# colinsongf/keyword_spotting

Hardware: NVIDIA B200
Metric: streamed audio-sec/sec, 2L GRU-128 KWS (higher is better)
Workload: dtype f16 operands / f32 accumulate+state

## Files before the change

keyword_spotting_b200/csrc/api.cu:

```cuda
#include <cmath>
#include <cstring>
#include <vector>

#include <cuda_fp16.h>

#include "common.cuh"

namespace kws {

static thread_local std::string g_last_error;

void set_error(const char* fmt, ...) {
  char buf[1024];
  va_list ap;
  va_start(ap, fmt);
  vsnprintf(buf, sizeof(buf), fmt, ap);
  va_end(ap);
  g_last_error = buf;
}
void clear_error() { g_last_error.clear(); }
int fail(int code, const char* fmt, ...) {
  char buf[1024];
  va_list ap;
  va_start(ap, fmt);
// ... 50 lines not shown
  if (m->aux_stream) cudaStreamDestroy(m->aux_stream);
  cudaFree(m->scratch_mel);
  cudaFree(m->scratch_seq);
  cudaFree(m->tc_xt);
  free_octbit(m);
  delete m;
}

}

using namespace kws;

extern "C" const char* kws_last_error(void) { return g_last_error.c_str(); }
extern "C" int kws_abi_version(void) { return KWS_B200_ABI_VERSION; }

extern "C" int kws_device_count(void) {
  clear_error();
  int n = 0;
  cudaError_t e = cudaGetDeviceCount(&n);
  if (e != cudaSuccess) return fail(KWS_ERR_CUDA, "cudaGetDeviceCount failed: %s", cudaGetErrorString(e));
  return n;
}

extern "C" int kws_model_create(const kws_model_config* cfg, const kws_model_weights* w, int device,
                                kws_model** out) {
  clear_error();
  KWS_REQUIRE(cfg && w && out, "NULL argument");
  *out = nullptr;
  KWS_REQUIRE(cfg->hidden == kHidden, "hidden_size must be %d (config/rnn_config.py:84)", kHidden);
  KWS_REQUIRE(cfg->num_layers >= 1 && cfg->num_layers <= kMaxLayers, "num_layers must be in [1, %d]", kMaxLayers);
  KWS_REQUIRE(cfg->num_classes >= 2 && cfg->num_classes <= kMaxClasses, "num_classes must be in [2, %d]", kMaxClasses);
  KWS_REQUIRE(cfg->n_mel >= 1 && cfg->n_mel <= kMaxMel, "n_mel must be in [1, %d]", kMaxMel);
  KWS_REQUIRE(cfg->fft_size == kFft && cfg->hop_size == kHop,
              "the front end is built for fft_size=%d hop_size=%d (config/rnn_config.py:57-58)", kFft, kHop);
  KWS_REQUIRE(w->mel_basis && w->fc_w && w->fc_b, "NULL weight pointer");
  for (int l = 0; l < cfg->num_layers; ++l)
    KWS_REQUIRE(w->gates_kernel[l] && w->gates_bias[l] && w->cand_kernel[l] && w->cand_bias[l],
                "NULL weight pointer for layer %d", l);
  int ndev = 0;
  cudaError_t e = cudaGetDeviceCount(&ndev);
  if (e != cudaSuccess || ndev <= 0)
    return fail(KWS_ERR_CUDA, "no CUDA device available (%s); libkws_b200 has no CPU fallback",
                e == cudaSuccess ? "device count 0" : cudaGetErrorString(e));
  KWS_REQUIRE(device >= 0 && device < ndev, "device %d out of range [0, %d)", device, ndev);
  KWS_CUDA_OK(cudaSetDevice(device));

  kws_model* m = new kws_model();
  m->cfg = *cfg;
  m->device = device;
  m->frontend = default_frontend();
  const int M = cfg->n_mel, H = kHidden, C = cfg->num_classes;
  int rc = upload(&m->mel_basis, w->mel_basis, static_cast<size_t>(kBins) * M);
  {
    std::vector<kws::MelQuad> quads;
    kws::build_mel_quads(w->mel_basis, M, &quads, &m->mel.quads_per_warp);
    if (rc == KWS_OK) rc = upload(&m->mel.quads, quads.data(), quads.size());
  }
  if (rc == KWS_OK) rc = build_frontend_tc_tables(m, w->mel_basis);
  std::vector<float2> tw(20 * 52);
  for (int k2 = 0; k2 < 20; ++k2)
    for (int j = 0; j < 52; ++j) {
      const double a = -2.0 * M_PI * static_cast<double>((j % 20) * k2) / kFft;
      tw[k2 * 52 + j] = make_float2(static_cast<float>(std::cos(a)), static_cast<float>(std::sin(a)));
    }
  if (rc == KWS_OK) rc = upload(&m->twiddle400, tw.data(), tw.size());
  for (int l = 0; l < cfg->num_layers && rc == KWS_OK; ++l) {
    const int in = l == 0 ? M : H;
    m->layer[l].in_dim = in;
    rc = upload(&m->layer[l].gates_kernel, w->gates_kernel[l], static_cast<size_t>(in + H) * 2 * H);
    if (rc == KWS_OK) rc = upload(&m->layer[l].gates_bias, w->gates_bias[l], 2 * H);
    if (rc == KWS_OK) rc = upload(&m->layer[l].cand_kernel, w->cand_kernel[l], static_cast<size_t>(in + H) * H);
    if (rc == KWS_OK) rc = upload(&m->layer[l].cand_bias, w->cand_bias[l], H);
    if (rc == KWS_OK) {
      std::vector<__half> packed;
      const bool last = l == cfg->num_layers - 1;
      const bool split = l == 0 && in <= 64 && gru_tc_can_split(in, last, device);
      if (l == 0 && !gru_tc_layer_fits(in, split, last, device)) m->tc_fits = false;
      pack_tc_weights(w->gates_kernel[l], w->cand_kernel[l], in, split, &packed, &m->layer[l].tc_kx, &m->layer[l].tc_kxw);
      __half* dptr = nullptr;
      rc = upload(&dptr, packed.data(), packed.size());
      m->layer[l].tc_wpack = dptr;
      std::vector<float> fused(3 * H);
      for (int i = 0; i < 2 * H; ++i) fused[i] = w->gates_bias[l][i];
      for (int i = 0; i < H; ++i) fused[2 * H + i] = w->cand_bias[l][i];
      if (rc == KWS_OK) rc = upload(&m->layer[l].tc_bias, fused.data(), fused.size());
    }
  }
  if (rc == KWS_OK) rc = upload(&m->fc_w, w->fc_w, static_cast<size_t>(H) * C);
  if (rc == KWS_OK) rc = upload(&m->fc_b, w->fc_b, C);
  m->fc_w_host.assign(w->fc_w, w->fc_w + static_cast<size_t>(H) * C);
  m->fc_b_host.assign(w->fc_b, w->fc_b + C);
  if (rc != KWS_OK) {
    free_model(m);
    return rc;
  }
  *out = m;
  return KWS_OK;
}

extern "C" int kws_model_destroy(kws_model* m) {
  clear_error();
  if (m) {
    cudaSetDevice(m->device);
    free_model(m);
  }
  return KWS_OK;
}

extern "C" int kws_model_set_precision(kws_model* m, int precision) {
  clear_error();
  KWS_REQUIRE(m != nullptr, "model is NULL");
  KWS_REQUIRE(precision == KWS_PRECISION_FP32 || precision == KWS_PRECISION_TC_FP16, "unknown precision %d", precision);
  m->precision = precision;
// ... 147 lines not shown
```

keyword_spotting_b200/csrc/common.cuh:

```cuda
#pragma once

#include <cuda_runtime.h>
#include <stdint.h>

#include <cstdarg>
#include <cstdio>
#include <string>
#include <vector>

#include "../../include/kws_b200.h"

namespace kws {

constexpr int kHidden = 128;
constexpr int kMaxLayers = 4;
constexpr int kMaxClasses = 16;
constexpr int kFft = 400;
constexpr int kHop = 160;
constexpr int kBins = kFft / 2 + 1;
constexpr int kMaxMel = 128;

void set_error(const char* fmt, ...);
void clear_error();
int fail(int code, const char* fmt, ...);
// ... 19 lines not shown
  } while (0)

inline int64_t ceil_div(int64_t a, int64_t b) { return (a + b - 1) / b; }

__host__ __device__ __forceinline__ int att_frames(int T, int combine) { return combine > 1 ? T / combine + 1 : T; }

constexpr int kAttCoreTcMaxKeys = 400;

struct AttLens {
  const int32_t* lens;
  int T;
  int combine;
  __device__ __forceinline__ int frames_in(long b) const { return lens ? min(max(__ldg(lens + b), 1), T) : T; }
  __device__ __forceinline__ int rows_of(long b) const { return att_frames(frames_in(b), combine); }
  __device__ __forceinline__ bool tile_live(int Tp, long rows, long r0, int tile) const {
    if (!lens) return true;
    const long b0 = r0 / Tp;
    const long rlast = (r0 + tile < rows ? r0 + tile : rows) - 1;
    return r0 - b0 * Tp < rows_of(b0) || (b0 + 1) * Tp <= rlast;
  }
};

int sm_count();

struct LayerWeights {
  int in_dim = 0;
  float* gates_kernel = nullptr;
  float* gates_bias = nullptr;
  float* cand_kernel = nullptr;
  float* cand_bias = nullptr;
  int tc_kx = 0;
  int tc_kxw = 0;
  void* tc_wpack = nullptr;
  float* tc_bias = nullptr;
};

struct OctbitMatrix {
  signed char* wq = nullptr;
  float* obias = nullptr;
  float scale = 0.0f;
  int* cand_count = nullptr;
  unsigned short* cand = nullptr;
  int B = 0, K = 0;
};

struct alignas(16) MelQuad {
  float w[4];
  int mag_off;
  int band_off;
  int pad[2];
};
struct MelSparse {
  MelQuad* quads = nullptr;
  int quads_per_warp = 0;
};

struct FrontendTcTables {
  bool ready = false;
  uint32_t* tw = nullptr;
  void* mel_seg = nullptr;
  float* mel_w = nullptr;
  int mel_nw = 0;
};

}

struct kws_model {
  kws_model_config cfg;
  int device = 0;
  int precision = KWS_PRECISION_TC_FP16;
  int frontend = KWS_FRONTEND_FFT;
  float* mel_basis = nullptr;
  kws::MelSparse mel;
  kws::FrontendTcTables fe_tc;
  float2* twiddle400 = nullptr;
  kws::LayerWeights layer[kws::kMaxLayers];
  float* fc_w = nullptr;
  float* fc_b = nullptr;
  std::vector<float> fc_w_host, fc_b_host;
  int64_t cap_streams = 0;
  int32_t cap_frames = 0;
  float* scratch_mel = nullptr;
  float* scratch_seq = nullptr;
  bool octbit = false;
  kws::OctbitMatrix oct_gates[kws::kMaxLayers], oct_cand[kws::kMaxLayers], oct_fc;
  float* oct_y_rows = nullptr;
  size_t oct_y_cap = 0;
  bool tc_fits = true;
  void* tc_xt = nullptr;
  size_t tc_xt_bytes = 0;
  cudaStream_t aux_stream = nullptr;
  std::vector<cudaEvent_t> aux_events;
};

namespace kws {

struct PcmSource {
  const void* body = nullptr;
  int64_t ld_body = 0;
  int32_t body_len = 0;
  int body_dtype = KWS_PCM_F32;
  const int16_t* head = nullptr;
  int64_t ld_head = 0;
  const int32_t* head_len = nullptr;
};

// ... 60 lines not shown
```

keyword_spotting_b200/csrc/fft400.cuh:

```cuda
#pragma once

#if defined(__CUDACC__)
#define KWS_HD __host__ __device__ __forceinline__
#else
#define KWS_HD inline
#endif

namespace kws {
namespace fft {

struct alignas(8) cpx {
  float re, im;
};

constexpr int kN = 400;
constexpr int kR = 20;
constexpr int kRowStride = 21;
constexpr int kBufSlots = kR * kRowStride;
constexpr int kPairWindow = 560;
constexpr int kBins = kN / 2 + 1;

#if defined(__CUDA_ARCH__)
KWS_HD float2 as_f2(cpx a) { return make_float2(a.re, a.im); }
KWS_HD cpx as_cpx(float2 a) { return cpx{a.x, a.y}; }
// ... 6 lines not shown
KWS_HD cpx cross_sq(cpx a, cpx b) {
  const float2 bs = make_float2(b.im, b.re);
  return as_cpx(__ffma2_rn(bs, bs, __fmul2_rn(as_f2(a), as_f2(a))));
}
#else
KWS_HD cpx cadd(cpx a, cpx b) { return cpx{a.re + b.re, a.im + b.im}; }
KWS_HD cpx csub(cpx a, cpx b) { return cpx{a.re - b.re, a.im - b.im}; }
KWS_HD cpx caxpy(float s, cpx b, cpx a) { return cpx{a.re + s * b.re, a.im + s * b.im}; }
KWS_HD cpx cscale(float s, cpx b) { return cpx{s * b.re, s * b.im}; }
KWS_HD cpx csub_i(cpx a, cpx b) { return cpx{a.re + b.im, a.im - b.re}; }
KWS_HD cpx cadd_i(cpx a, cpx b) { return cpx{a.re - b.im, a.im + b.re}; }
KWS_HD cpx cross_sq(cpx a, cpx b) { return cpx{a.re * a.re + b.im * b.im, a.im * a.im + b.re * b.re}; }
#endif
KWS_HD cpx cmul(cpx a, cpx b) { return cpx{a.re * b.re - a.im * b.im, a.re * b.im + a.im * b.re}; }

KWS_HD void dft4(cpx& a0, cpx& a1, cpx& a2, cpx& a3) {
  const cpx t0 = cadd(a0, a2), t1 = csub(a0, a2), t2 = cadd(a1, a3), t3 = csub(a1, a3);
  a0 = cadd(t0, t2);
  a2 = csub(t0, t2);
  a1 = csub_i(t1, t3);
  a3 = cadd_i(t1, t3);
}

KWS_HD void dft5(cpx& a0, cpx& a1, cpx& a2, cpx& a3, cpx& a4) {
  const float c1 = 0.30901699437494742f;
  const float c2 = -0.80901699437494742f;
  const float s1 = 0.95105651629515357f;
  const float s2 = 0.58778525229247313f;
  const cpx t1 = cadd(a1, a4), t2 = cadd(a2, a3), t3 = csub(a1, a4), t4 = csub(a2, a3);
  const cpx m1 = caxpy(c2, t2, caxpy(c1, t1, a0));
  const cpx m2 = caxpy(c1, t2, caxpy(c2, t1, a0));
  const cpx n1 = caxpy(s2, t4, cscale(s1, t3));
  const cpx n2 = caxpy(-s1, t4, cscale(s2, t3));
  a0 = cadd(cadd(a0, t1), t2);
  a1 = csub_i(m1, n1);
  a4 = cadd_i(m1, n1);
  a2 = csub_i(m2, n2);
  a3 = cadd_i(m2, n2);
}

KWS_HD constexpr int pfa_slot(int k) { return (5 * (k % 4) + 4 * (k % 5)) % 20; }

KWS_HD void dft20_pfa(cpx (&v)[20]) {
#pragma unroll
  for (int n2 = 0; n2 < 5; ++n2)
    dft4(v[(4 * n2) % 20], v[(5 + 4 * n2) % 20], v[(10 + 4 * n2) % 20], v[(15 + 4 * n2) % 20]);
#pragma unroll
  for (int k1 = 0; k1 < 4; ++k1)
    dft5(v[(5 * k1) % 20], v[(5 * k1 + 4) % 20], v[(5 * k1 + 8) % 20], v[(5 * k1 + 12) % 20],
         v[(5 * k1 + 16) % 20]);
}

constexpr int kTwStride = 52;
constexpr int kTwSlots = kR * kTwStride;
KWS_HD constexpr int tw_base(int warp, int lane) { return (12 * warp) % kR + lane; }

KWS_HD void stage1_col(int n1, cpx (&v)[20], const cpx* tw, cpx* buf) {
  dft20_pfa(v);
  buf[n1 * kRowStride] = v[pfa_slot(0)];
#pragma unroll
  for (int k2 = 1; k2 < kR; ++k2) buf[n1 * kRowStride + k2] = cmul(v[pfa_slot(k2)], tw[k2 * kTwStride]);
}

KWS_HD void stage2_col(int k2, cpx* buf, cpx (&v)[20]) {
#pragma unroll
  for (int n1 = 0; n1 < kR; ++n1) v[n1] = buf[n1 * kRowStride + k2];
  dft20_pfa(v);
#pragma unroll
  for (int k1 = kR / 2; k1 < kR; ++k1) buf[k1 * kRowStride + k2] = v[pfa_slot(k1)];
}

KWS_HD float sqrt_fast(float x) {
#if defined(__CUDA_ARCH__)
  float r;
  asm("sqrt.approx.ftz.f32 %0, %1;" : "=f"(r) : "f"(x));
  return r;
#else
  return __builtin_sqrtf(x);
#endif
}

KWS_HD void untangle_col(int k2, const cpx (&v)[20], const cpx* buf, float* mag_a, float* mag_b, int k1_stride) {
  const int mcol = k2 == 0 ? 0 : kR - k2;
  const int mrow0 = k2 == 0 ? kR : kR - 1;
#pragma unroll
  for (int k1 = 0; k1 < kR / 2; ++k1) {
    const cpx zk = v[pfa_slot(k1)];
    int mrow = mrow0 - k1;
    const bool self = mrow == kR;
    if (self) mrow = kR - 1;
    cpx zm = buf[mrow * kRowStride + mcol];
    if (self) zm = zk;
    const cpx sp = cadd(zk, zm), sm = csub(zk, zm);
    const cpx sq = cross_sq(sp, sm);
    mag_a[k1 * k1_stride] = sqrt_fast(sq.re);
    mag_b[k1 * k1_stride] = sqrt_fast(sq.im);
  }
  if (k2 == 0) {
    const cpx z = v[pfa_slot(kR / 2)];
    mag_a[(kR / 2) * k1_stride] = 2.0f * (z.re < 0.0f ? -z.re : z.re);
    mag_b[(kR / 2) * k1_stride] = 2.0f * (z.im < 0.0f ? -z.im : z.im);
  }
}

}
}
```

keyword_spotting_b200/csrc/frontend.cu:

```cuda
#include <algorithm>
#include <cstring>
#include <vector>

#include "common.cuh"
#include "tc05.cuh"
#include "fft400.cuh"

namespace kws {

using fft::cpx;

constexpr int kFePairs = 16;
constexpr int kFeThreads = kFePairs * fft::kR;
constexpr int kFeWarps = kFeThreads / 32;
constexpr int kFeItemFrames = 2 * kFePairs;
constexpr int kFeBlock = 2 * kHop;
constexpr int kFeSkew = 20;
constexpr int kFeWinSamples = kFePairs * kFeBlock + (kFft - kHop);
constexpr int kFeWinRounds = (kFeWinSamples + kFeThreads - 1) / kFeThreads;
constexpr int kFeQuadRounds = (kFeWinSamples + 4 * kFeThreads - 1) / (4 * kFeThreads);
constexpr int kFeLastQuads = (kFeWinSamples - 4 * kFeThreads * (kFeQuadRounds - 1)) / 4;
static_assert(kFeWinSamples % 4 == 0 && kFeBlock % 4 == 0, "quads must not straddle a skew boundary");
constexpr int kFeQuadSmemMax = 512;
constexpr int kFeItemHop = kFePairs * kFeBlock;
constexpr int kFeMagStride = 66;
constexpr int kFeWinFloats = kFeWinRounds * (kFeBlock + kFeSkew);
constexpr int kFeMagRows = (fft::kBins + 3) / 2;
constexpr int kFeMagFloats = kFeMagRows * kFeMagStride;
constexpr int kFeMagLive = (fft::kBins / 2) * kFeMagStride;
constexpr int kFeRegionFloats = kFeMagFloats > kFeWinFloats ? kFeMagFloats : kFeWinFloats;
static_assert(kFeWinFloats <= kFeMagLive, "the window must not reach the rows that hold the zero bins");
static_assert((kFeRegionFloats * 4) % 16 == 0, "mel quads follow the region and are read as float4");

struct FrontendParams {
  PcmSource src;
  long S;
  int max_frames;
  int groups;
  const int* nframes;
  int n_mel;
  const cpx* twiddle;
  const MelQuad* mel_q;
  int mel_qpw;
  int vec_ok;
  float* mel_out;
  int tiled_out;
  int tile_chunks;
  int tile_split;
  unsigned c_magic;
  unsigned q_magic;
  float mag_scale;
  int fuse_pre;
  long long vad_limit;
  int16_t* tail_next;
  int* len_next;
  unsigned char* silence;
  int* nframes_out;
};

__device__ __forceinline__ int mag_slot(int pair, int fr) { return ((10 * pair) & 15) + 16 * (pair >> 3) + fr; }
__device__ __forceinline__ int slot_frame(int slot) {
  const int pair = ((5 * ((slot & 15) >> 1)) & 7) + 8 * (slot >> 4);
  return 2 * pair + (slot & 1);
}
__device__ __forceinline__ int mag_index(int bin, int slot) { return (bin >> 1) * kFeMagStride + 2 * slot + (bin & 1); }

__device__ __forceinline__ float4 quad_to_float(uint2 q) {
  return make_float4(static_cast<float>(static_cast<short>(q.x & 0xffffu)), static_cast<float>(static_cast<short>(q.x >> 16)),
                     static_cast<float>(static_cast<short>(q.y & 0xffffu)), static_cast<float>(static_cast<short>(q.y >> 16)));
}

template <bool kQuadsInSmem>
__global__ void __launch_bounds__(kFeThreads, 2)
frontend_kernel(const FrontendParams p) {
  extern __shared__ __align__(16) unsigned char smem_raw[];
  cpx* twp = reinterpret_cast<cpx*>(smem_raw);
  cpx* buf = twp + fft::kTwSlots;
  float* win = reinterpret_cast<float*>(buf + kFePairs * fft::kBufSlots);
  int* red = reinterpret_cast<int*>(win + kFeRegionFloats);
  MelQuad* s_q = reinterpret_cast<MelQuad*>(red + 16);

  const int tid = threadIdx.x, warp = tid >> 5, lane = tid & 31;
  for (int i = tid; i < fft::kTwSlots; i += kFeThreads) twp[i] = p.twiddle[i];
  if (kQuadsInSmem) {
    const int n16 = kFeWarps * p.mel_qpw * static_cast<int>(sizeof(MelQuad) / 16);
    for (int i = tid; i < n16; i += kFeThreads) reinterpret_cast<uint4*>(s_q)[i] = reinterpret_cast<const uint4*>(p.mel_q)[i];
  }
  for (int i = kFeMagLive + tid; i < kFeRegionFloats; i += kFeThreads) win[i] = 0.0f;

  const int pair = tid / fft::kR;
  const int col = tid - pair * fft::kR;
  cpx* my_buf = buf + pair * fft::kBufSlots;
  const float* my_win = win + pair * (kFeBlock + kFeSkew) + col;
  const cpx* my_tw = twp + fft::tw_base(warp, lane);
  float* out_tile = reinterpret_cast<float*>(buf);
  const long items = p.S * p.groups;
  const bool items32 = items < (1L << 32);
  auto stream_of = [&](long item) -> long {
    if (p.groups == 1) return item;
    if (items32) return static_cast<long>(static_cast<unsigned>(item) / static_cast<unsigned>(p.groups));
    return item / p.groups;
  };
  const bool i16 = p.src.body_dtype == KWS_PCM_I16;
  const int M = p.n_mel;
  const int Mp = M | 1;
  const MelQuad* my_q = (kQuadsInSmem ? s_q : p.mel_q) + warp * p.mel_qpw;
  __syncthreads();

  const bool last_quad_ok = tid < kFeLastQuads;
  auto load_quads = [&](long item, int head_len, uint2 (&pre)[kFeQuadRounds]) {
    const long s = stream_of(item);
    const int q0 = static_cast<int>(item - s * p.groups) * kFeItemHop;
    const int total_len = head_len + p.src.body_len;
    const int16_t* body = static_cast<const int16_t*>(p.src.body) + s * p.src.ld_body - head_len;
    const int16_t* head = p.src.head + s * p.src.ld_head;
    if (p.vec_ok && ((head_len | total_len) & 3) == 0) {
#pragma unroll
      for (int r = 0; r < kFeQuadRounds; ++r) {
        const int q = q0 + 4 * tid + 4 * kFeThreads * r;
        const int16_t* src = (r == 0 && q < head_len ? head : body) + q;
        uint2 v = make_uint2(0u, 0u);
        if (q < total_len && (r < kFeQuadRounds - 1 || last_quad_ok)) v = __ldg(reinterpret_cast<const uint2*>(src));
        pre[r] = v;
      }
    } else {
      auto fetch1 = [&](int q) -> unsigned {
        int x = 0;
        if (q < head_len) x = head[q];
        else if (q < total_len) x = body[q];
        return static_cast<unsigned>(x) & 0xffffu;
      };
#pragma unroll 1
      for (int r = 0; r < kFeQuadRounds; ++r) {
        const int q = q0 + 4 * tid + 4 * kFeThreads * r;
        uint2 v = make_uint2(0u, 0u);
        if (q < total_len && (r < kFeQuadRounds - 1 || last_quad_ok))
          v = make_uint2(fetch1(q) | (fetch1(q + 1) << 16), fetch1(q + 2) | (fetch1(q + 3) << 16));
        if (r == 0) pre[0] = v;
        if (r == 1) pre[1] = v;
        if (r == 2) pre[2] = v;
        if (r == 3) pre[3] = v;
        if (r == 4) pre[4] = v;
      }
    }
  };
  static_assert(kFeQuadRounds == 5, "load_quads' element-wise path names the rounds");
  float* my_stage = win + 4 * tid + kFeSkew * (tid / (kFeBlock / 4));
  auto store_quads = [&](int q0, int head_len, const uint2 (&pre)[kFeQuadRounds]) {
    float4 f[kFeQuadRounds];
#pragma unroll
    for (int r = 0; r < kFeQuadRounds; ++r) {
      f[r] = quad_to_float(pre[r]);
      if (r < kFeQuadRounds - 1 || last_quad_ok) *reinterpret_cast<float4*>(my_stage + (4 * kFeThreads + 4 * kFeSkew) * r) = f[r];
    }
    if (!p.fuse_pre) return 0;
    float acc = 0.0f;
#pragma unroll
    for (int r = 1; r < kFeQuadRounds; ++r) acc += (fabsf(f[r].x) + fabsf(f[r].y)) + (fabsf(f[r].z) + fabsf(f[r].w));
    const int q = q0 + 4 * tid;
    acc += (q >= head_len ? fabsf(f[0].x) : 0.0f) + (q + 1 >= head_len ? fabsf(f[0].y) : 0.0f) +
           (q + 2 >= head_len ? fabsf(f[0].z) : 0.0f) + (q + 3 >= head_len ? fabsf(f[0].w) : 0.0f);
    return static_cast<int>(acc);
  };

  long item = blockIdx.x;
  uint2 pre[kFeQuadRounds];
  int head_len = 0;
  if (i16 && item < items) {
    head_len = p.src.head_len ? p.src.head_len[stream_of(item)] : 0;
    load_quads(item, head_len, pre);
  }

  for (; item < items; item += gridDim.x) {
    const long s = stream_of(item);
    const int g = static_cast<int>(item - s * p.groups);
    if (!i16) head_len = p.src.head_len ? p.src.head_len[s] : 0;
    const int total_len = head_len + p.src.body_len;
    const int nfr_sig = total_len >= kFft ? 1 + (total_len - kFft) / kHop : 0;
    int nfr = p.fuse_pre ? nfr_sig : (p.nframes ? p.nframes[s] : nfr_sig);
    if (nfr > p.max_frames) nfr = p.max_frames;
    const int q0 = g * kFeItemHop;
    const int f0 = g * kFeItemFrames;
    const long next = item + gridDim.x;
    int head_len_next = 0;
    if (i16 && next < items && p.src.head_len) head_len_next = p.src.head_len[stream_of(next)];

    int vad_acc = 0;
    if (i16) {
      vad_acc = store_quads(q0, head_len, pre);
    } else {
      const bool last_ok = tid < kFeWinSamples - kFeBlock * (kFeWinRounds - 1);
      const float* body = static_cast<const float*>(p.src.body) + s * p.src.ld_body + q0 + tid;
#pragma unroll
      for (int r = 0; r < kFeWinRounds; ++r) {
        const int q = q0 + tid + kFeBlock * r;
        const float v = q < total_len ? __ldg(body + kFeBlock * r) : 0.0f;
        if (r < kFeWinRounds - 1 || last_ok) win[tid + (kFeBlock + kFeSkew) * r] = v;
      }
    }
    if (p.fuse_pre) {
      vad_acc = __reduce_add_sync(0xffffffffu, vad_acc);
      if (lane == 0) red[warp] = vad_acc;
    }
    __syncthreads();

    if (p.fuse_pre) {
      const int keep = total_len >= kFft ? (total_len - kFft) % kHop + (kFft - kHop) : total_len;
      const int start = total_len - keep;
      int16_t* tnext = p.tail_next + s * 400;
      if (((start | keep) & 3) == 0 && (reinterpret_cast<uintptr_t>(p.tail_next) & 7) == 0) {
        if (4 * tid < keep) {
          const int w = start + 4 * tid;
          const float4 f = *reinterpret_cast<const float4*>(win + w + kFeSkew * (w / kFeBlock));
          const unsigned lo = (static_cast<unsigned>(__float2int_rn(f.x)) & 0xffffu) | (static_cast<unsigned>(__float2int_rn(f.y)) << 16);
          const unsigned hi = (static_cast<unsigned>(__float2int_rn(f.z)) & 0xffffu) | (static_cast<unsigned>(__float2int_rn(f.w)) << 16);
          *reinterpret_cast<uint2*>(tnext + 4 * tid) = make_uint2(lo, hi);
        }
      } else {
        for (int i = tid; i < keep; i += kFeThreads) {
          const int w = start + i;
          tnext[i] = static_cast<int16_t>(win[w + kFeSkew * (w / kFeBlock)]);
        }
      }
      if (warp == 0) {
        const int part = lane < kFeWarps ? red[lane] : 0;
        const int sum = __reduce_add_sync(0xffffffffu, part);
        if (lane == 0) {
          p.silence[s] = static_cast<long long>(sum) > p.vad_limit ? 0 : 1;
          p.nframes_out[s] = nfr;
          p.len_next[s] = keep;
        }
      }
    }

    const int fa = f0 + 2 * pair;
    const bool live = fa < nfr;
    cpx v[20];
    if (live) {
#pragma unroll
      for (int n2 = 0; n2 < 20; ++n2) {
        v[n2].re = my_win[20 * n2 + (n2 >= 16 ? kFeSkew : 0)];
        v[n2].im = my_win[kHop + 20 * n2 + (n2 >= 8 ? kFeSkew : 0)];
      }
      fft::stage1_col(col, v, my_tw, my_buf);
    }
    __syncthreads();
    if (live) fft::stage2_col(col, my_buf, v);
    __syncthreads();
    float* mag = win;
    if (live)
      fft::untangle_col(col, v, my_buf, mag + mag_index(col, mag_slot(pair, 0)), mag + mag_index(col, mag_slot(pair, 1)),
                        (fft::kR / 2) * kFeMagStride);
    __syncthreads();
    if (i16 && next < items) load_quads(next, head_len_next, pre);
    {
      char* orow = reinterpret_cast<char*>(out_tile + slot_frame(lane) * Mp);
      const char* mcol = reinterpret_cast<const char*>(mag + 2 * lane);
      const float scale = p.mag_scale;
      const MelQuad* rec = my_q;
      float2 acc = make_float2(0.0f, 0.0f);
      auto fetch = [&](const MelQuad* r, float4& w4, int2& me) {
        if (kQuadsInSmem) {
          w4 = *reinterpret_cast<const float4*>(r->w);
          me = *reinterpret_cast<const int2*>(&r->mag_off);
        } else {
          w4 = __ldg(reinterpret_cast<const float4*>(r->w));
          me = __ldg(reinterpret_cast<const int2*>(&r->mag_off));
        }
      };
      auto apply = [&](const float4& w4, const int2& me, const float2& m01, const float2& m23) {
        acc = __ffma2_rn(m01, make_float2(w4.x, w4.y), acc);
        acc = __ffma2_rn(m23, make_float2(w4.z, w4.w), acc);
        if (me.y >= 0) {
          *reinterpret_cast<float*>(orow + me.y) = (acc.x + acc.y) * scale;
          acc = make_float2(0.0f, 0.0f);
        }
      };
#pragma unroll 1
      for (int q = p.mel_qpw; q > 0; q -= 2, rec += 2) {
        float4 wa, wb;
        int2 ma, mb;
        fetch(rec, wa, ma);
        fetch(rec + 1, wb, mb);
        const float2 a01 = *reinterpret_cast<const float2*>(mcol + ma.x);
        const float2 a23 = *reinterpret_cast<const float2*>(mcol + ma.x + kFeMagStride * sizeof(float));
        const float2 b01 = *reinterpret_cast<const float2*>(mcol + mb.x);
        const float2 b23 = *reinterpret_cast<const float2*>(mcol + mb.x + kFeMagStride * sizeof(float));
        apply(wa, ma, a01, a23);
        apply(wb, mb, b01, b23);
      }
    }
    __syncthreads();
    {
      int nfi = nfr - f0;
      if (nfi > kFeItemFrames) nfi = kFeItemFrames;
      const int total = nfi > 0 ? nfi * M : 0;
      if (p.tiled_out) {
        const int nc = p.tile_chunks;
        const int per_frame = p.tile_split ? 2 * nc : nc;
        uint4* dst = reinterpret_cast<uint4*>(p.mel_out) + ((s >> 7) * p.max_frames + f0) * static_cast<long>(per_frame) * 128 + (s & 127);
        const int pieces = nfi > 0 ? nfi * nc : 0;
        for (int i = tid; i < pieces; i += kFeThreads) {
          const int f = nc == 1 ? i : static_cast<int>(__umulhi(static_cast<unsigned>(i), p.c_magic));
          const int c = i - f * nc;
          const float* src = out_tile + f * Mp + 8 * c;
          float v[8];
#pragma unroll
          for (int j = 0; j < 8; ++j) v[j] = 8 * c + j < M ? src[j] : 0.0f;
          uint4 hi, lo;
          tc::split_half8(v, &hi, &lo);
          dst[(f * per_frame + c) * 128] = hi;
          if (p.tile_split) dst[(f * per_frame + nc + c) * 128] = lo;
        }
      } else if ((M & 3) == 0 && (reinterpret_cast<uintptr_t>(p.mel_out) & 15) == 0) {
        const int Q = M >> 2;
        float4* dst4 = reinterpret_cast<float4*>(p.mel_out) + (s * p.max_frames + f0) * static_cast<long>(Q);
        for (int i = tid; i < (total >> 2); i += kFeThreads) {
          const int f = Q == 1 ? i : static_cast<int>(__umulhi(static_cast<unsigned>(i), p.q_magic));
          const int c = i - f * Q;
          const float* src = out_tile + f * Mp + 4 * c;
          dst4[i] = make_float4(src[0], src[1], src[2], src[3]);
        }
      } else {
        float* dst = p.mel_out + (s * p.max_frames + f0) * M;
        for (int i = tid; i < total; i += kFeThreads) {
          const int f = i / M;
          dst[i] = out_tile[f * Mp + (i - f * M)];
        }
      }
    }
    head_len = head_len_next;
  }
}

void build_mel_quads(const float* basis, int M, std::vector<MelQuad>* quads, int* quads_per_warp) {
  struct Band { int b, lo, nq; };
  std::vector<Band> bands;
  for (int b = 0; b < M; ++b) {
    int lo = -1, hi = -1;
    for (int k = 0; k < kBins; ++k)
      if (basis[static_cast<size_t>(k) * M + b] != 0.0f) {
        if (lo < 0) lo = k;
        hi = k;
      }
    if (lo < 0) lo = hi = 0;
    lo &= ~1;
    bands.push_back(Band{b, lo, (hi - lo + 1 + 3) / 4});
  }
  std::stable_sort(bands.begin(), bands.end(), [](const Band& x, const Band& y) { return x.nq > y.nq; });
  std::vector<std::vector<Band>> per_warp(kFeWarps);
  std::vector<int> load(kFeWarps, 0);
  for (const Band& bd : bands) {
    const int w = static_cast<int>(std::min_element(load.begin(), load.end()) - load.begin());
    per_warp[w].push_back(bd);
    load[w] += bd.nq;
  }
  const int qpw = (std::max(1, *std::max_element(load.begin(), load.end())) + 1) & ~1;
  MelQuad zero;
  zero.w[0] = zero.w[1] = zero.w[2] = zero.w[3] = 0.0f;
  zero.mag_off = 0;
  zero.band_off = -1;
  zero.pad[0] = zero.pad[1] = 0;
  quads->assign(static_cast<size_t>(kFeWarps) * qpw, zero);
  for (int w = 0; w < kFeWarps; ++w) {
    size_t at = static_cast<size_t>(w) * qpw;
    for (const Band& bd : per_warp[w])
      for (int j = 0; j < bd.nq; ++j, ++at) {
        MelQuad& q = (*quads)[at];
        for (int e = 0; e < 4; ++e) {
          const int k = bd.lo + 4 * j + e;
          q.w[e] = k < kBins ? basis[static_cast<size_t>(k) * M + bd.b] : 0.0f;
        }
        q.mag_off = ((bd.lo + 4 * j) / 2) * kFeMagStride * static_cast<int>(sizeof(float));
        q.band_off = j == bd.nq - 1 ? bd.b * static_cast<int>(sizeof(float)) : -1;
      }
  }
  *quads_per_warp = qpw;
}

static bool quads_in_smem(const kws_model* m) { return kFeWarps * m->mel.quads_per_warp <= kFeQuadSmemMax; }
static size_t frontend_smem_bytes(const kws_model* m) {
  return sizeof(cpx) * fft::kTwSlots + sizeof(cpx) * kFePairs * fft::kBufSlots + sizeof(float) * kFeRegionFloats +
         sizeof(int) * 16 + (quads_in_smem(m) ? sizeof(MelQuad) * kFeWarps * m->mel.quads_per_warp : 0);
}

bool frontend_can_fuse_pre(const kws_model* m, int chunk_len, int tail_cap) {
  if (frontend_uses_tc(m, KWS_PCM_I16)) return chunk_len + tail_cap - 1 <= kFft + kHop * (frontend_tc_item_frames() - 1) + kHop - 1;
  return chunk_len + tail_cap - 1 <= kFeWinSamples;
}

int launch_frontend(const kws_model* m, const PcmSource& src, int64_t S, int32_t max_frames,
                    const int32_t* nframes, float* mel_out, cudaStream_t st, const FrontendPre* pre, bool tiled_out) {
  if (S <= 0) return KWS_OK;
  if (max_frames <= 0 && !pre) return KWS_OK;
  if (frontend_uses_tc(m, src.body_dtype)) return launch_frontend_tc(m, src, S, max_frames, nframes, mel_out, st, pre, tiled_out);
  FrontendParams p;
  p.src = src;
  p.S = S;
  p.max_frames = max_frames;
  p.groups = static_cast<int>(ceil_div(max_frames > 0 ? max_frames : 1, kFeItemFrames));
  p.nframes = nframes;
  p.n_mel = m->cfg.n_mel;
  p.twiddle = reinterpret_cast<const cpx*>(m->twiddle400);
  p.mel_q = m->mel.quads;
  p.mel_qpw = m->mel.quads_per_warp;
  p.vec_ok = (reinterpret_cast<uintptr_t>(src.body) % 8 == 0 && src.ld_body % 4 == 0 &&
              reinterpret_cast<uintptr_t>(src.head) % 8 == 0 && src.ld_head % 4 == 0) ? 1 : 0;
  p.mel_out = mel_out;
  p.tiled_out = tiled_out ? 1 : 0;
  p.q_magic = m->cfg.n_mel >= 4 ? static_cast<unsigned>(((1ull << 32) + (m->cfg.n_mel / 4) - 1) / (m->cfg.n_mel / 4)) : 0u;
  p.tile_chunks = tiled_out ? mel_tile_chunks(m) : 1;
  p.tile_split = tiled_out && mel_tile_split(m) ? 1 : 0;
  p.c_magic = static_cast<unsigned>(((1ull << 32) + p.tile_chunks - 1) / p.tile_chunks);
  p.mag_scale = src.body_dtype == KWS_PCM_I16 ? 0.5f / 32768.0f : 0.5f;
  p.fuse_pre = 0;
  p.vad_limit = 0;
  p.tail_next = nullptr;
  p.len_next = nullptr;
  p.silence = nullptr;
  p.nframes_out = nullptr;
  if (pre) {
    if (p.groups != 1 || src.body_dtype != KWS_PCM_I16)
      return fail(KWS_ERR_INVALID_ARGUMENT, "fused pre-step needs an int16 chunk that fits one work item");
    p.fuse_pre = 1;
    p.vad_limit = pre->vad_limit;
    p.tail_next = pre->tail_next;
    p.len_next = pre->len_next;
    p.silence = pre->silence;
    p.nframes_out = pre->nframes_out;
  }
  const bool in_smem = quads_in_smem(m);
  auto kernel = in_smem ? frontend_kernel<true> : frontend_kernel<false>;
  const size_t smem = frontend_smem_bytes(m);
  KWS_CUDA_OK(cudaFuncSetAttribute(kernel, cudaFuncAttributeMaxDynamicSharedMemorySize, static_cast<int>(smem)));
  int per_sm = 0;
  KWS_CUDA_OK(cudaOccupancyMaxActiveBlocksPerMultiprocessor(&per_sm, kernel, kFeThreads, smem));
  if (per_sm < 1) return fail(KWS_ERR_CUDA, "frontend_kernel does not fit on an SM (smem %zu)", smem);
  const long items = S * p.groups;
  long blocks = items;
  const long resident = static_cast<long>(per_sm) * sm_count();
  if (blocks > resident) blocks = resident;
  kernel<<<static_cast<unsigned>(blocks), kFeThreads, smem, st>>>(p);
  KWS_LAUNCH_OK("frontend_kernel");
  return KWS_OK;
}

}

extern "C" int kws_debug_mel_quads(const float* basis, int n_mel, int* quads_out, int capacity) {
  kws::clear_error();
  if (!basis || n_mel < 1 || n_mel > kws::kMaxMel) return kws::fail(KWS_ERR_INVALID_ARGUMENT, "bad basis / n_mel");
  std::vector<kws::MelQuad> quads;
  int qpw = 0;
  kws::build_mel_quads(basis, n_mel, &quads, &qpw);
  static_assert(sizeof(kws::MelQuad) == 32, "record layout");
  const int n = static_cast<int>(quads.size());
  if (quads_out) {
    if (capacity < n) return kws::fail(KWS_ERR_INVALID_ARGUMENT, "capacity %d < %d quads", capacity, n);
    memcpy(quads_out, quads.data(), sizeof(kws::MelQuad) * n);
  }
  return qpw;
}
```

Baseline: 9.145 million.

## Pass mel quads as grid-constant param and specialise frontend kernel on dtype

```diff
diff --git a/keyword_spotting_b200/csrc/api.cu b/keyword_spotting_b200/csrc/api.cu
--- a/keyword_spotting_b200/csrc/api.cu
+++ b/keyword_spotting_b200/csrc/api.cu
@@ -126,13 +126,13 @@
   const int M = cfg->n_mel, H = kHidden, C = cfg->num_classes;
   int rc = upload(&m->mel_basis, w->mel_basis, static_cast<size_t>(kBins) * M);
   {
-    std::vector<kws::MelQuad> quads;
+    std::vector<kws::MelQuad>& quads = m->mel.quads_host;
     kws::build_mel_quads(w->mel_basis, M, &quads, &m->mel.quads_per_warp);
     if (rc == KWS_OK) rc = upload(&m->mel.quads, quads.data(), quads.size());
   }
   if (rc == KWS_OK) rc = build_frontend_tc_tables(m, w->mel_basis);
-  std::vector<float2> tw(20 * 52);
-  for (int k2 = 0; k2 < 20; ++k2)
+  std::vector<float2> tw(21 * 52);
+  for (int k2 = 0; k2 < 21; ++k2)
     for (int j = 0; j < 52; ++j) {
       const double a = -2.0 * M_PI * static_cast<double>((j % 20) * k2) / kFft;
       tw[k2 * 52 + j] = make_float2(static_cast<float>(std::cos(a)), static_cast<float>(std::sin(a)));
diff --git a/keyword_spotting_b200/csrc/common.cuh b/keyword_spotting_b200/csrc/common.cuh
--- a/keyword_spotting_b200/csrc/common.cuh
+++ b/keyword_spotting_b200/csrc/common.cuh
@@ -95,6 +95,7 @@
 };
 struct MelSparse {
   MelQuad* quads = nullptr;
+  std::vector<MelQuad> quads_host;
   int quads_per_warp = 0;
 };
 
diff --git a/keyword_spotting_b200/csrc/fft400.cuh b/keyword_spotting_b200/csrc/fft400.cuh
--- a/keyword_spotting_b200/csrc/fft400.cuh
+++ b/keyword_spotting_b200/csrc/fft400.cuh
@@ -82,14 +82,30 @@
 }
 
 constexpr int kTwStride = 52;
+constexpr int kTwRows = kR + 1;
 constexpr int kTwSlots = kR * kTwStride;
 KWS_HD constexpr int tw_base(int warp, int lane) { return (12 * warp) % kR + lane; }
+constexpr int kTwHeld = kR / 2;
+
+KWS_HD cpx mirror_twiddle(cpx w20, cpx t) {
+  return cpx{fmaf(w20.re, t.re, w20.im * t.im), fmaf(w20.im, t.re, -(w20.re * t.im))};
+}
 
 KWS_HD void stage1_col(int n1, cpx (&v)[20], const cpx* tw, cpx* buf) {
   dft20_pfa(v);
   buf[n1 * kRowStride] = v[pfa_slot(0)];
 #pragma unroll
   for (int k2 = 1; k2 < kR; ++k2) buf[n1 * kRowStride + k2] = cmul(v[pfa_slot(k2)], tw[k2 * kTwStride]);
+}
+
+KWS_HD void stage1_col(int n1, cpx (&v)[20], const cpx (&tw)[kTwHeld], cpx w20, cpx* buf) {
+  dft20_pfa(v);
+  buf[n1 * kRowStride] = v[pfa_slot(0)];
+#pragma unroll
+  for (int k2 = 1; k2 <= kTwHeld; ++k2) buf[n1 * kRowStride + k2] = cmul(v[pfa_slot(k2)], tw[k2 - 1]);
+#pragma unroll
+  for (int k2 = kTwHeld + 1; k2 < kR; ++k2)
+    buf[n1 * kRowStride + k2] = cmul(v[pfa_slot(k2)], mirror_twiddle(w20, tw[kR - k2 - 1]));
 }
 
 KWS_HD void stage2_col(int k2, cpx* buf, cpx (&v)[20]) {
diff --git a/keyword_spotting_b200/csrc/frontend.cu b/keyword_spotting_b200/csrc/frontend.cu
--- a/keyword_spotting_b200/csrc/frontend.cu
+++ b/keyword_spotting_b200/csrc/frontend.cu
@@ -5,6 +5,16 @@
 #include "common.cuh"
 #include "tc05.cuh"
 #include "fft400.cuh"
+
+#ifndef KWS_FE_TW_REGS
+#define KWS_FE_TW_REGS 0
+#endif
+#ifndef KWS_FE_QUAD_PARAM
+#define KWS_FE_QUAD_PARAM 1
+#endif
+#ifndef KWS_FE_PAIR_WIN
+#define KWS_FE_PAIR_WIN 0
+#endif
 
 namespace kws {
 
@@ -21,7 +31,15 @@
 constexpr int kFeQuadRounds = (kFeWinSamples + 4 * kFeThreads - 1) / (4 * kFeThreads);
 constexpr int kFeLastQuads = (kFeWinSamples - 4 * kFeThreads * (kFeQuadRounds - 1)) / 4;
 static_assert(kFeWinSamples % 4 == 0 && kFeBlock % 4 == 0, "quads must not straddle a skew boundary");
-constexpr int kFeQuadSmemMax = 512;
+constexpr int kFePairWords = kFeWinSamples - kHop;
+constexpr int kFeSegQuads = kHop / 4;
+constexpr int kFeSegGroups = kFeThreads / kFeSegQuads;
+constexpr int kFeSegsPerGroup = 4;
+constexpr int kFeLoadRounds = kFeSegsPerGroup + 2;
+static_assert(kFeSegGroups * kFeSegQuads == kFeThreads && kFeBlock == 2 * kHop, "segment groups");
+static_assert((kFeSegGroups - 1) * kFeSegsPerGroup + kFeLoadRounds - 1 == kFeWinSamples / kHop, "group 7 ends at x segment 33");
+static_assert(kFft <= 3 * kHop, "the carried tail (< 400 samples) lies in segments 0..2 (group 0, rounds 0..2)");
+constexpr int kFeQuadFastMax = 512;
 constexpr int kFeItemHop = kFePairs * kFeBlock;
 constexpr int kFeMagStride = 66;
 constexpr int kFeWinFloats = kFeWinRounds * (kFeBlock + kFeSkew);
@@ -31,6 +49,13 @@
 constexpr int kFeRegionFloats = kFeMagFloats > kFeWinFloats ? kFeMagFloats : kFeWinFloats;
 static_assert(kFeWinFloats <= kFeMagLive, "the window must not reach the rows that hold the zero bins");
 static_assert((kFeRegionFloats * 4) % 16 == 0, "mel quads follow the region and are read as float4");
+constexpr int kFeTwSmemSlots = KWS_FE_TW_REGS ? 0 : fft::kTwSlots;
+
+template <int kN>
+struct MelQuadBlock {
+  MelQuad q[kN];
+};
+constexpr int kFeQuadParamCap = KWS_FE_QUAD_PARAM ? kFeQuadFastMax : 1;
 
 struct FrontendParams {
   PcmSource src;
@@ -64,35 +89,51 @@
   return 2 * pair + (slot & 1);
 }
 __device__ __forceinline__ int mag_index(int bin, int slot) { return (bin >> 1) * kFeMagStride + 2 * slot + (bin & 1); }
+__device__ __forceinline__ int win_pos(int i) { return i + kFeSkew * (i / kFeBlock); }
 
 __device__ __forceinline__ float4 quad_to_float(uint2 q) {
   return make_float4(static_cast<float>(static_cast<short>(q.x & 0xffffu)), static_cast<float>(static_cast<short>(q.x >> 16)),
                      static_cast<float>(static_cast<short>(q.y & 0xffffu)), static_cast<float>(static_cast<short>(q.y >> 16)));
 }
-
-template <bool kQuadsInSmem>
+__device__ __forceinline__ int abs_pair(unsigned w) { return abs(static_cast<int>(static_cast<short>(w & 0xffffu))) + abs(static_cast<int>(w) >> 16); }
+__device__ __forceinline__ cpx pair_to_cpx(unsigned w) {
+  const float2 f = make_float2(__uint_as_float(__byte_perm(w, 0x4b000000u, 0x7410)), __uint_as_float(__byte_perm(w, 0x4b000000u, 0x7432)));
+  const float2 x = __fadd2_rn(f, make_float2(-8421376.0f, -8421376.0f));
+  return cpx{x.x, x.y};
+}
+
+template <bool kQuadsFast, bool kI16>
 __global__ void __launch_bounds__(kFeThreads, 2)
-frontend_kernel(const FrontendParams p) {
+frontend_kernel(const FrontendParams p, const __grid_constant__ MelQuadBlock<kQuadsFast ? kFeQuadParamCap : 1> qb) {
+  constexpr bool kPairWin = kI16 && KWS_FE_PAIR_WIN;
   extern __shared__ __align__(16) unsigned char smem_raw[];
   cpx* twp = reinterpret_cast<cpx*>(smem_raw);
-  cpx* buf = twp + fft::kTwSlots;
+  cpx* buf = twp + kFeTwSmemSlots;
   float* win = reinterpret_cast<float*>(buf + kFePairs * fft::kBufSlots);
   int* red = reinterpret_cast<int*>(win + kFeRegionFloats);
   MelQuad* s_q = reinterpret_cast<MelQuad*>(red + 16);
+  constexpr bool kQuadsInSmem = kQuadsFast && !KWS_FE_QUAD_PARAM;
 
   const int tid = threadIdx.x, warp = tid >> 5, lane = tid & 31;
+  const int pair = tid / fft::kR;
+  const int col = tid - pair * fft::kR;
+#if KWS_FE_TW_REGS
+  cpx tw[fft::kTwHeld];
+#pragma unroll
+  for (int k = 0; k < fft::kTwHeld; ++k) tw[k] = p.twiddle[(k + 1) * fft::kTwStride + col];
+  const cpx w20 = p.twiddle[fft::kR * fft::kTwStride + col];
+#else
   for (int i = tid; i < fft::kTwSlots; i += kFeThreads) twp[i] = p.twiddle[i];
+  const cpx* my_tw = twp + fft::tw_base(warp, lane);
+#endif
   if (kQuadsInSmem) {
     const int n16 = kFeWarps * p.mel_qpw * static_cast<int>(sizeof(MelQuad) / 16);
     for (int i = tid; i < n16; i += kFeThreads) reinterpret_cast<uint4*>(s_q)[i] = reinterpret_cast<const uint4*>(p.mel_q)[i];
   }
   for (int i = kFeMagLive + tid; i < kFeRegionFloats; i += kFeThreads) win[i] = 0.0f;
 
-  const int pair = tid / fft::kR;
-  const int col = tid - pair * fft::kR;
   cpx* my_buf = buf + pair * fft::kBufSlots;
   const float* my_win = win + pair * (kFeBlock + kFeSkew) + col;
-  const cpx* my_tw = twp + fft::tw_base(warp, lane);
   float* out_tile = reinterpret_cast<float*>(buf);
   const long items = p.S * p.groups;
   const bool items32 = items < (1L << 32);
@@ -101,14 +142,22 @@
     if (items32) return static_cast<long>(static_cast<unsigned>(item) / static_cast<unsigned>(p.groups));
     return item / p.groups;
   };
-  const bool i16 = p.src.body_dtype == KWS_PCM_I16;
   const int M = p.n_mel;
   const int Mp = M | 1;
-  const MelQuad* my_q = (kQuadsInSmem ? s_q : p.mel_q) + warp * p.mel_qpw;
+  const int q_first = __reduce_max_sync(0xffffffffu, warp) * p.mel_qpw;
   __syncthreads();
 
+  constexpr int kRounds = kPairWin ? kFeLoadRounds : kFeQuadRounds;
+  const int seg_group = tid / kFeSegQuads;
+  const bool last_group = seg_group == kFeSegGroups - 1;
+  const int seg_off = kFeSegsPerGroup * kHop * seg_group + 4 * (tid - seg_group * kFeSegQuads);
   const bool last_quad_ok = tid < kFeLastQuads;
-  auto load_quads = [&](long item, int head_len, uint2 (&pre)[kFeQuadRounds]) {
+  auto window_sample = [&](int r) { return kPairWin ? seg_off + kHop * r : 4 * tid + 4 * kFeThreads * r; };
+  auto round_ok = [&](int r) {
+    if (kPairWin) return (r < kFeLoadRounds - 1 || last_group) && seg_off + kHop * r < kFeWinSamples;
+    return r < kFeQuadRounds - 1 || last_quad_ok;
+  };
+  auto load_quads = [&](long item, int head_len, uint2 (&pre)[kRounds]) {
     const long s = stream_of(item);
     const int q0 = static_cast<int>(item - s * p.groups) * kFeItemHop;
     const int total_len = head_len + p.src.body_len;
@@ -116,11 +165,11 @@
     const int16_t* head = p.src.head + s * p.src.ld_head;
     if (p.vec_ok && ((head_len | total_len) & 3) == 0) {
 #pragma unroll
-      for (int r = 0; r < kFeQuadRounds; ++r) {
-        const int q = q0 + 4 * tid + 4 * kFeThreads * r;
-        const int16_t* src = (r == 0 && q < head_len ? head : body) + q;
+      for (int r = 0; r < kRounds; ++r) {
+        const int q = q0 + window_sample(r);
+        const int16_t* src = ((kPairWin ? r < 3 : r == 0) && q < head_len ? head : body) + q;
         uint2 v = make_uint2(0u, 0u);
-        if (q < total_len && (r < kFeQuadRounds - 1 || last_quad_ok)) v = __ldg(reinterpret_cast<const uint2*>(src));
+        if (q < total_len && round_ok(r)) v = __ldg(reinterpret_cast<const uint2*>(src));
         pre[r] = v;
       }
     } else {
@@ -131,22 +180,51 @@
         return static_cast<unsigned>(x) & 0xffffu;
       };
 #pragma unroll 1
-      for (int r = 0; r < kFeQuadRounds; ++r) {
-        const int q = q0 + 4 * tid + 4 * kFeThreads * r;
+      for (int r = 0; r < kRounds; ++r) {
+        const int q = q0 + window_sample(r);
         uint2 v = make_uint2(0u, 0u);
-        if (q < total_len && (r < kFeQuadRounds - 1 || last_quad_ok))
+        if (q < total_len && round_ok(r))
           v = make_uint2(fetch1(q) | (fetch1(q + 1) << 16), fetch1(q + 2) | (fetch1(q + 3) << 16));
         if (r == 0) pre[0] = v;
         if (r == 1) pre[1] = v;
         if (r == 2) pre[2] = v;
         if (r == 3) pre[3] = v;
         if (r == 4) pre[4] = v;
+        if (kRounds > 5 && r == 5) pre[kRounds - 1] = v;
       }
     }
   };
-  static_assert(kFeQuadRounds == 5, "load_quads' element-wise path names the rounds");
+  static_assert(kFeQuadRounds == 5 && kFeLoadRounds == 6, "load_quads' element-wise path names the rounds");
   float* my_stage = win + 4 * tid + kFeSkew * (tid / (kFeBlock / 4));
-  auto store_quads = [&](int q0, int head_len, const uint2 (&pre)[kFeQuadRounds]) {
+  unsigned* my_pairs = reinterpret_cast<unsigned*>(win) + seg_off + 2 * kFeSkew * seg_group;
+  auto store_quads = [&](int q0, int head_len, const uint2 (&pre)[kRounds]) {
+    if constexpr (kPairWin) {
+#pragma unroll
+      for (int r = 0; r < kFeLoadRounds - 1; ++r) {
+        if ((r < kFeSegsPerGroup || last_group) && seg_off + kHop * r < kFePairWords) {
+          const unsigned lx = pre[r].x ^ 0x80008000u, ly = pre[r].y ^ 0x80008000u;
+          const unsigned hx = pre[r + 1].x ^ 0x80008000u, hy = pre[r + 1].y ^ 0x80008000u;
+          *reinterpret_cast<uint4*>(my_pairs + kHop * r + kFeSkew * (r >> 1)) =
+              make_uint4(__byte_perm(lx, hx, 0x5410), __byte_perm(lx, hx, 0x7632), __byte_perm(ly, hy, 0x5410), __byte_perm(ly, hy, 0x7632));
+        }
+      }
+      if (!p.fuse_pre) return 0;
+      int acc = 0;
+#pragma unroll
+      for (int r = 0; r < kFeLoadRounds; ++r) {
+        if (!(r < kFeSegsPerGroup || last_group)) continue;
+        const int q = q0 + seg_off + kHop * r;
+        if (r < 3) {
+          acc += (q >= head_len ? abs(static_cast<int>(static_cast<short>(pre[r].x & 0xffffu))) : 0) +
+                 (q + 1 >= head_len ? abs(static_cast<int>(pre[r].x) >> 16) : 0) +
+                 (q + 2 >= head_len ? abs(static_cast<int>(static_cast<short>(pre[r].y & 0xffffu))) : 0) +
+                 (q + 3 >= head_len ? abs(static_cast<int>(pre[r].y) >> 16) : 0);
+        } else {
+          acc += abs_pair(pre[r].x) + abs_pair(pre[r].y);
+        }
+      }
+      return acc;
+    } else {
     float4 f[kFeQuadRounds];
 #pragma unroll
     for (int r = 0; r < kFeQuadRounds; ++r) {
@@ -161,12 +239,32 @@
     acc += (q >= head_len ? fabsf(f[0].x) : 0.0f) + (q + 1 >= head_len ? fabsf(f[0].y) : 0.0f) +
            (q + 2 >= head_len ? fabsf(f[0].z) : 0.0f) + (q + 3 >= head_len ? fabsf(f[0].w) : 0.0f);
     return static_cast<int>(acc);
+    }
   };
+  auto staged_quad = [&](int w) -> uint2 {
+    if constexpr (kPairWin) {
+      const bool lo = w < kFePairWords;
+      const uint4 u = *reinterpret_cast<const uint4*>(reinterpret_cast<const unsigned*>(win) + win_pos(lo ? w : w - kHop));
+      const unsigned sel = lo ? 0x5410u : 0x7632u;
+      return make_uint2(__byte_perm(u.x, u.y, sel) ^ 0x80008000u, __byte_perm(u.z, u.w, sel) ^ 0x80008000u);
+    }
+    const float4 f = *reinterpret_cast<const float4*>(win + win_pos(w));
+    return make_uint2((static_cast<unsigned>(__float2int_rn(f.x)) & 0xffffu) | (static_cast<unsigned>(__float2int_rn(f.y)) << 16),
+                      (static_cast<unsigned>(__float2int_rn(f.z)) & 0xffffu) | (static_cast<unsigned>(__float2int_rn(f.w)) << 16));
+  };
+  auto staged_sample = [&](int w) -> int16_t {
+    if constexpr (kPairWin) {
+      const bool lo = w < kFePairWords;
+      const unsigned u = reinterpret_cast<const unsigned*>(win)[win_pos(lo ? w : w - kHop)];
+      return static_cast<int16_t>((lo ? u : u >> 16) ^ 0x8000u);
+    }
+    return static_cast<int16_t>(win[win_pos(w)]);
+  };
 
   long item = blockIdx.x;
-  uint2 pre[kFeQuadRounds];
+  uint2 pre[kRounds];
   int head_len = 0;
-  if (i16 && item < items) {
+  if (kI16 && item < items) {
     head_len = p.src.head_len ? p.src.head_len[stream_of(item)] : 0;
     load_quads(item, head_len, pre);
   }
@@ -174,7 +272,7 @@
   for (; item < items; item += gridDim.x) {
     const long s = stream_of(item);
     const int g = static_cast<int>(item - s * p.groups);
-    if (!i16) head_len = p.src.head_len ? p.src.head_len[s] : 0;
+    if (!kI16) head_len = p.src.head_len ? p.src.head_len[s] : 0;
     const int total_len = head_len + p.src.body_len;
     const int nfr_sig = total_len >= kFft ? 1 + (total_len - kFft) / kHop : 0;
     int nfr = p.fuse_pre ? nfr_sig : (p.nframes ? p.nframes[s] : nfr_sig);
@@ -183,10 +281,10 @@
     const int f0 = g * kFeItemFrames;
     const long next = item + gridDim.x;
     int head_len_next = 0;
-    if (i16 && next < items && p.src.head_len) head_len_next = p.src.head_len[stream_of(next)];
+    if (kI16 && next < items && p.src.head_len) head_len_next = p.src.head_len[stream_of(next)];
 
     int vad_acc = 0;
-    if (i16) {
+    if (kI16) {
       vad_acc = store_quads(q0, head_len, pre);
     } else {
       const bool last_ok = tid < kFeWinSamples - kFeBlock * (kFeWinRounds - 1);
@@ -204,23 +302,14 @@
     }
     __syncthreads();
 
-    if (p.fuse_pre) {
+    if (kI16 && p.fuse_pre) {
       const int keep = total_len >= kFft ? (total_len - kFft) % kHop + (kFft - kHop) : total_len;
       const int start = total_len - keep;
       int16_t* tnext = p.tail_next + s * 400;
       if (((start | keep) & 3) == 0 && (reinterpret_cast<uintptr_t>(p.tail_next) & 7) == 0) {
-        if (4 * tid < keep) {
-          const int w = start + 4 * tid;
-          const float4 f = *reinterpret_cast<const float4*>(win + w + kFeSkew * (w / kFeBlock));
-          const unsigned lo = (static_cast<unsigned>(__float2int_rn(f.x)) & 0xffffu) | (static_cast<unsigned>(__float2int_rn(f.y)) << 16);
-          const unsigned hi = (static_cast<unsigned>(__float2int_rn(f.z)) & 0xffffu) | (static_cast<unsigned>(__float2int_rn(f.w)) << 16);
-          *reinterpret_cast<uint2*>(tnext + 4 * tid) = make_uint2(lo, hi);
-        }
+        if (4 * tid < keep) *reinterpret_cast<uint2*>(tnext + 4 * tid) = staged_quad(start + 4 * tid);
       } else {
-        for (int i = tid; i < keep; i += kFeThreads) {
-          const int w = start + i;
-          tnext[i] = static_cast<int16_t>(win[w + kFeSkew * (w / kFeBlock)]);
-        }
+        for (int i = tid; i < keep; i += kFeThreads) tnext[i] = staged_sample(start + i);
       }
       if (warp == 0) {
         const int part = lane < kFeWarps ? red[lane] : 0;
@@ -237,12 +326,24 @@
     const bool live = fa < nfr;
     cpx v[20];
     if (live) {
-#pragma unroll
-      for (int n2 = 0; n2 < 20; ++n2) {
-        v[n2].re = my_win[20 * n2 + (n2 >= 16 ? kFeSkew : 0)];
-        v[n2].im = my_win[kHop + 20 * n2 + (n2 >= 8 ? kFeSkew : 0)];
-      }
+      if constexpr (kPairWin) {
+        const unsigned* my_pw = reinterpret_cast<const unsigned*>(my_win);
+#pragma unroll
+        for (int n2 = 0; n2 < 20; ++n2) v[n2] = pair_to_cpx(my_pw[20 * n2 + (n2 >= 16 ? kFeSkew : 0)]);
+      } else {
+#pragma unroll
+        for (int n2 = 0; n2 < 20; ++n2) {
+          v[n2].re = my_win[20 * n2 + (n2 >= 16 ? kFeSkew : 0)];
+          v[n2].im = my_win[kHop + 20 * n2 + (n2 >= 8 ? kFeSkew : 0)];
+        }
+      }
+#if KWS_FE_TW_REGS
+      cpx w20_item = w20;
+      asm volatile("" : "+f"(w20_item.re), "+f"(w20_item.im));
+      fft::stage1_col(col, v, tw, w20_item, my_buf);
+#else
       fft::stage1_col(col, v, my_tw, my_buf);
+#endif
     }
     __syncthreads();
     if (live) fft::stage2_col(col, my_buf, v);
@@ -252,20 +353,23 @@
       fft::untangle_col(col, v, my_buf, mag + mag_index(col, mag_slot(pair, 0)), mag + mag_index(col, mag_slot(pair, 1)),
                         (fft::kR / 2) * kFeMagStride);
     __syncthreads();
-    if (i16 && next < items) load_quads(next, head_len_next, pre);
+    if (kI16 && next < items) load_quads(next, head_len_next, pre);
     {
       char* orow = reinterpret_cast<char*>(out_tile + slot_frame(lane) * Mp);
       const char* mcol = reinterpret_cast<const char*>(mag + 2 * lane);
       const float scale = p.mag_scale;
-      const MelQuad* rec = my_q;
       float2 acc = make_float2(0.0f, 0.0f);
-      auto fetch = [&](const MelQuad* r, float4& w4, int2& me) {
+      auto fetch = [&](int i, float4& w4, int2& me) {
         if (kQuadsInSmem) {
-          w4 = *reinterpret_cast<const float4*>(r->w);
-          me = *reinterpret_cast<const int2*>(&r->mag_off);
+          w4 = *reinterpret_cast<const float4*>(s_q[i].w);
+          me = *reinterpret_cast<const int2*>(&s_q[i].mag_off);
+        } else if (kQuadsFast) {
+          const MelQuad& r = qb.q[i];
+          w4 = make_float4(r.w[0], r.w[1], r.w[2], r.w[3]);
+          me = make_int2(r.mag_off, r.band_off);
         } else {
-          w4 = __ldg(reinterpret_cast<const float4*>(r->w));
-          me = __ldg(reinterpret_cast<const int2*>(&r->mag_off));
+          w4 = __ldg(reinterpret_cast<const float4*>(p.mel_q[i].w));
+          me = __ldg(reinterpret_cast<const int2*>(&p.mel_q[i].mag_off));
         }
       };
       auto apply = [&](const float4& w4, const int2& me, const float2& m01, const float2& m23) {
@@ -277,11 +381,11 @@
         }
       };
 #pragma unroll 1
-      for (int q = p.mel_qpw; q > 0; q -= 2, rec += 2) {
+      for (int i = q_first; i < q_first + p.mel_qpw; i += 2) {
         float4 wa, wb;
         int2 ma, mb;
-        fetch(rec, wa, ma);
-        fetch(rec + 1, wb, mb);
+        fetch(i, wa, ma);
+        fetch(i + 1, wb, mb);
         const float2 a01 = *reinterpret_cast<const float2*>(mcol + ma.x);
         const float2 a23 = *reinterpret_cast<const float2*>(mcol + ma.x + kFeMagStride * sizeof(float));
         const float2 b01 = *reinterpret_cast<const float2*>(mcol + mb.x);
@@ -378,15 +482,34 @@
   *quads_per_warp = qpw;
 }
 
-static bool quads_in_smem(const kws_model* m) { return kFeWarps * m->mel.quads_per_warp <= kFeQuadSmemMax; }
+static bool quads_fast(const kws_model* m) { return kFeWarps * m->mel.quads_per_warp <= kFeQuadFastMax; }
 static size_t frontend_smem_bytes(const kws_model* m) {
-  return sizeof(cpx) * fft::kTwSlots + sizeof(cpx) * kFePairs * fft::kBufSlots + sizeof(float) * kFeRegionFloats +
-         sizeof(int) * 16 + (quads_in_smem(m) ? sizeof(MelQuad) * kFeWarps * m->mel.quads_per_warp : 0);
+  return sizeof(cpx) * kFeTwSmemSlots + sizeof(cpx) * kFePairs * fft::kBufSlots + sizeof(float) * kFeRegionFloats +
+         sizeof(int) * 16 + (!KWS_FE_QUAD_PARAM && quads_fast(m) ? sizeof(MelQuad) * kFeWarps * m->mel.quads_per_warp : 0);
 }
 
 bool frontend_can_fuse_pre(const kws_model* m, int chunk_len, int tail_cap) {
   if (frontend_uses_tc(m, KWS_PCM_I16)) return chunk_len + tail_cap - 1 <= kFft + kHop * (frontend_tc_item_frames() - 1) + kHop - 1;
   return chunk_len + tail_cap - 1 <= kFeWinSamples;
+}
+
+template <bool kQuadsFast, bool kI16>
+static int launch_frontend_kernel(const kws_model* m, const FrontendParams& p, long items, cudaStream_t st) {
+  auto kernel = frontend_kernel<kQuadsFast, kI16>;
+  MelQuadBlock<kQuadsFast ? kFeQuadParamCap : 1> qb{};
+  if (kQuadsFast && KWS_FE_QUAD_PARAM)
+    memcpy(qb.q, m->mel.quads_host.data(), sizeof(MelQuad) * m->mel.quads_host.size());
+  const size_t smem = frontend_smem_bytes(m);
+  KWS_CUDA_OK(cudaFuncSetAttribute(kernel, cudaFuncAttributeMaxDynamicSharedMemorySize, static_cast<int>(smem)));
+  int per_sm = 0;
+  KWS_CUDA_OK(cudaOccupancyMaxActiveBlocksPerMultiprocessor(&per_sm, kernel, kFeThreads, smem));
+  if (per_sm < 1) return fail(KWS_ERR_CUDA, "frontend_kernel does not fit on an SM (smem %zu)", smem);
+  long blocks = items;
+  const long resident = static_cast<long>(per_sm) * sm_count();
+  if (blocks > resident) blocks = resident;
+  kernel<<<static_cast<unsigned>(blocks), kFeThreads, smem, st>>>(p, qb);
+  KWS_LAUNCH_OK("frontend_kernel");
+  return KWS_OK;
 }
 
 int launch_frontend(const kws_model* m, const PcmSource& src, int64_t S, int32_t max_frames,
@@ -429,20 +552,11 @@
     p.silence = pre->silence;
     p.nframes_out = pre->nframes_out;
   }
-  const bool in_smem = quads_in_smem(m);
-  auto kernel = in_smem ? frontend_kernel<true> : frontend_kernel<false>;
-  const size_t smem = frontend_smem_bytes(m);
-  KWS_CUDA_OK(cudaFuncSetAttribute(kernel, cudaFuncAttributeMaxDynamicSharedMemorySize, static_cast<int>(smem)));
-  int per_sm = 0;
-  KWS_CUDA_OK(cudaOccupancyMaxActiveBlocksPerMultiprocessor(&per_sm, kernel, kFeThreads, smem));
-  if (per_sm < 1) return fail(KWS_ERR_CUDA, "frontend_kernel does not fit on an SM (smem %zu)", smem);
   const long items = S * p.groups;
-  long blocks = items;
-  const long resident = static_cast<long>(per_sm) * sm_count();
-  if (blocks > resident) blocks = resident;
-  kernel<<<static_cast<unsigned>(blocks), kFeThreads, smem, st>>>(p);
-  KWS_LAUNCH_OK("frontend_kernel");
-  return KWS_OK;
+  const bool i16 = src.body_dtype == KWS_PCM_I16;
+  if (quads_fast(m))
+    return i16 ? launch_frontend_kernel<true, true>(m, p, items, st) : launch_frontend_kernel<true, false>(m, p, items, st);
+  return i16 ? launch_frontend_kernel<false, true>(m, p, items, st) : launch_frontend_kernel<false, false>(m, p, items, st);
 }
 
 }
```

Result: no change. 9.218 million (median of 6 runs) (+0.8%).
